# d8ahazard/AudioLab

Measured on AMD Instinct MI355X. Metric: stems*realtime-factor (44.1kHz stereo), higher is better.
Workload: dtype bf16; 1 GPU; MDX-Net UVR 4-stem (4x TFC-TDF U-Net L=11 g=48 dim_f=3072 dim_t=256 n_fft=6144), 300 s 44.1 kHz stereo in total, margin chunker, windows/launch=52; stems=4

## Files before the change

### audiolab_amd/csrc/tdfnet.hip

```cpp
#include "mma.h"
#include <alsep_gfx950_asm.h>

#include <map>

namespace {

constexpr int kThreads = 256;

template <typename T> struct Vec16;
template <> struct Vec16<float> { static constexpr int N = 4; };
template <> struct Vec16<bf16_t> { static constexpr int N = 8; };
__device__ __forceinline__ void store_vec(float* p, const float* y) { *reinterpret_cast<float4*>(p) = make_float4(y[0], y[1], y[2], y[3]); }
__device__ __forceinline__ void store_vec(bf16_t* p, const float* y) {
    bf16x8 q;
#pragma unroll
    for (int e = 0; e < 8; ++e) q[e] = (bf16_t)y[e];
    *reinterpret_cast<bf16x8*>(p) = q;
}
__device__ __forceinline__ void load_vec(const float* p, float* x) {
    const float4 q = *reinterpret_cast<const float4*>(p);
    x[0] = q.x; x[1] = q.y; x[2] = q.z; x[3] = q.w;
}
__device__ __forceinline__ void load_vec(const bf16_t* p, float* x) {
    const bf16x8 q = *reinterpret_cast<const bf16x8*>(p);
#pragma unroll
    for (int e = 0; e < 8; ++e) x[e] = (float)q[e];
}

constexpr int kFirstThreads = 192;
template <typename T>
__global__ void __launch_bounds__(kFirstThreads)
first_conv_kernel(const T* __restrict__ X, T* __restrict__ Y, const float* __restrict__ W,
                  const float* __restrict__ scale, const float* __restrict__ shift, int64_t npix, int g,
                  float in_scale) {
    constexpr int VN = Vec16<T>::N;
    const int q = g / VN;
    const int ppb = kFirstThreads / q;
    const int tg = threadIdx.x % q, tp = threadIdx.x / q;
    if (tp >= ppb) return;
    const int co = tg * VN;
    float4 w[VN];
    float sc[VN], sh[VN];
#pragma unroll
    for (int r = 0; r < VN; ++r) {
        w[r] = *reinterpret_cast<const float4*>(W + (co + r) * 4);
        sc[r] = scale[co + r] * in_scale;
        sh[r] = shift[co + r];
    }
    for (int64_t p = (int64_t)blockIdx.x * ppb + tp; p < npix; p += (int64_t)gridDim.x * ppb) {
        float x[4];
        load4(X + p * 4, x);
        float y[VN];
#pragma unroll
        for (int r = 0; r < VN; ++r) {
            float a = w[r].x * x[0];
            a = fmaf(w[r].y, x[1], a);
            a = fmaf(w[r].z, x[2], a);
            a = fmaf(w[r].w, x[3], a);
            y[r] = fmaxf(fmaf(a, sc[r], sh[r]), 0.f);
        }
        store_vec(Y + p * g + co, y);
    }
}

template <typename T>
__global__ void __launch_bounds__(kThreads)
final_conv_kernel(const T* __restrict__ X, T* __restrict__ Y, const float* __restrict__ W,
                  const float* __restrict__ bias, int64_t npix, int c, float alpha, float beta) {
    constexpr int VN = Vec16<T>::N;
    const int lane = threadIdx.x & 63, wave = threadIdx.x >> 6;
    const int gpp = c / VN;
    T* stg = reinterpret_cast<T*>(alsep_smem) + (size_t)wave * 64 * c;
    const int64_t p0 = ((int64_t)blockIdx.x * 4 + wave) * 64;
    for (int i = lane; i < 64 * gpp; i += 64) {
        const int64_t pix = p0 + i / gpp;
        vec16 v = zero16();
        if (pix < npix) v = *reinterpret_cast<const vec16*>(X + p0 * c + (int64_t)i * VN);
        *reinterpret_cast<vec16*>(stg + (size_t)i * VN) = v;
    }
    __builtin_amdgcn_wave_barrier();
    const int64_t p = p0 + lane;
    float y[4] = {bias[0], bias[1], bias[2], bias[3]};
    for (int ci = 0; ci < c; ci += VN) {
        float x[VN];
        load_vec(stg + (size_t)lane * c + ci, x);
#pragma unroll
// ... 1423 lines not shown
            wait_vmcnt<GLDS_PER_TILE>();                     \
        } else {                                                                                  \
            wait_vmcnt<0>();                                                                      \
        }                                                                                         \
        barrier_nodrain();                                        \
        compute(S_);                                                                              \
        barrier_nodrain();                                   \
    } while (0)
    issue(0, 0);
    for (int it = 0; it < ntile; it += 2) {
        ALSEP_TDF_STEP(it, 0);
        if (it + 1 < ntile) ALSEP_TDF_STEP(it + 1, 1);
    }
#undef ALSEP_TDF_STEP
    float* stg = reinterpret_cast<float*>(alsep_smem) + (size_t)wave * (64 * Tc::SS);
    float bvv[8];
#pragma unroll
    for (int mi = 0; mi < 8; ++mi) {
        const int fo = row0 + mi * 16 + l15;
        bvv[mi] = (bias && fo < M) ? bias[fo] : 0.f;
    }
    float sc[3][4], sh[3][4];
#pragma unroll
    for (int ni = 0; ni < 3; ++ni)
#pragma unroll
        for (int r = 0; r < 4; ++r) {
            sc[ni][r] = uvalid ? scale[cb + ni * 16 + 4 * lq + r] : 0.f;
            sh[ni][r] = uvalid ? shift[cb + ni * 16 + 4 * lq + r] : 0.f;
        }
#pragma unroll
    for (int half = 0; half < 2; ++half) {
#pragma unroll
        for (int ni = 0; ni < 3; ++ni)
#pragma unroll
            for (int m4 = 0; m4 < 4; ++m4) {
                const int mi = half * 4 + m4;
                float4 v;
                v.x = fmaxf(fmaf(acc[ni][mi][0] + bvv[mi], sc[ni][0], sh[ni][0]), 0.f);
                v.y = fmaxf(fmaf(acc[ni][mi][1] + bvv[mi], sc[ni][1], sh[ni][1]), 0.f);
                v.z = fmaxf(fmaf(acc[ni][mi][2] + bvv[mi], sc[ni][2], sh[ni][2]), 0.f);
                v.w = fmaxf(fmaf(acc[ni][mi][3] + bvv[mi], sc[ni][3], sh[ni][3]), 0.f);
                *reinterpret_cast<float4*>(stg + (m4 * 16 + l15) * Tc::SS + ni * 16 + 4 * lq) = v;
            }
        __builtin_amdgcn_wave_barrier();
#pragma unroll
        for (int it = 0; it < 6; ++it) {
            const int gidx = it * 64 + lane;
            const int fr = gidx / 6, cg = gidx % 6;
            const int fo = row0 + half * 64 + fr;
            const float4 lo = *reinterpret_cast<const float4*>(stg + fr * Tc::SS + cg * 8);
            const float4 hi = *reinterpret_cast<const float4*>(stg + fr * Tc::SS + cg * 8 + 4);
            if (uvalid && fo < M) {
                const int64_t o = (bt * M + fo) * (int64_t)C + cb + cg * 8;
                float y[8] = {lo.x, lo.y, lo.z, lo.w, hi.x, hi.y, hi.z, hi.w};
                if (RESIDUAL) {
                    const bf16x8 xr = *reinterpret_cast<const bf16x8*>(R + o);
#pragma unroll
                    for (int e = 0; e < 8; ++e) y[e] += (float)xr[e];
                }
                bf16x8 q;
#pragma unroll
                for (int e = 0; e < 8; ++e) q[e] = (bf16_t)y[e];
                stream_store(reinterpret_cast<bf16x8*>(Y + o), q);
            }
        }
        __builtin_amdgcn_wave_barrier();
    }
}

template <int WM>
struct TdfWide {
    static constexpr int TR = 48, BM = TR * WM, UN = 4, UC = 48, BK = 64, NST = 3;
    static constexpr int THREADS = 64 * WM;
    static constexpr int UNIT_ELEMS = BK * UC;
    static constexpr int STAGE_ELEMS = UN * UNIT_ELEMS;
    static constexpr int PIECES = STAGE_ELEMS / 8 / 64;
    static constexpr int GLDS = PIECES / WM;
    static constexpr int WLOADS = 6;
    static constexpr size_t ring_bytes = (size_t)NST * STAGE_ELEMS * sizeof(bf16_t);
    static constexpr int SS = 52;
    static constexpr size_t stage_bytes = (size_t)WM * TR * SS * sizeof(float);
    static constexpr size_t lds_bytes = ring_bytes > stage_bytes ? ring_bytes : stage_bytes;
    static_assert(PIECES % WM == 0 && 6 % GLDS == 0, "a wave's LDS-DMA pieces stay inside one unit");
};

template <int OFF>
__device__ __forceinline__ bf16x8 tdfw_read_frag(const bf16_t* base) {
    const bf16x4 lo = lds_read_tr16_b64_off<OFF>(base);
    const bf16x4 hi = lds_read_tr16_b64_off<OFF + 16 * 48 * 2>(base);
    return __builtin_shufflevector(lo, hi, 0, 1, 2, 3, 4, 5, 6, 7);
}
template <int KS, int U>
__device__ __forceinline__ void tdfw_read_x(bf16x8 (&xf)[3], const bf16_t* base) {
    constexpr int OFF = (U * 64 * 48 + KS * 32 * 48) * 2;
    xf[0] = tdfw_read_frag<OFF>(base);
    xf[1] = tdfw_read_frag<OFF + 32>(base);
    xf[2] = tdfw_read_frag<OFF + 64>(base);
}

#ifndef ALSEP_TDF_ABL
#define ALSEP_TDF_ABL 0
#endif
template <int WM, bool RESIDUAL, int RPF = 2>
__global__ void __launch_bounds__(64 * WM, 2)
tdf_bf16_wide_kernel(const bf16_t* __restrict__ X, bf16_t* __restrict__ Y, const bf16_t* __restrict__ Wf,
                     const float* __restrict__ bias, const float* __restrict__ scale, const float* __restrict__ shift,
                     const bf16_t* __restrict__ R, int M, int K, int64_t nunits, int C, int nyb) {
    typedef TdfWide<WM> Tc;
    bf16_t* ring = reinterpret_cast<bf16_t*>(alsep_smem);
    const int tid = threadIdx.x, lane = tid & 63;
    const int wave = __builtin_amdgcn_readfirstlane(tid >> 6);
    const int l15 = lane & 15, lq = lane >> 4;
    int bx = blockIdx.x, by = blockIdx.y;
    if (nyb > 0) {
        const int i = (int)blockIdx.x >> 3;
        by = i % nyb;
        bx = (i / nyb) * 8 + ((int)blockIdx.x & 7);
    }
    const int rowblk = by * WM + wave;
    const int upc = C / Tc::UC;
    const int64_t u0 = (int64_t)bx * Tc::UN;
    const int ntile = K / Tc::BK;
    if (ntile <= 0) return;

    const int du = (wave * Tc::GLDS) / 6, dp0 = (wave * Tc::GLDS) % 6;
    const int64_t dU = u0 + du;
    const char* xu = reinterpret_cast<const char*>(X + ((dU / upc) * K) * (int64_t)C + (int)(dU % upc) * Tc::UC) +
                     (size_t)(dp0 / 3) * 32 * C * sizeof(bf16_t);
    unsigned xoff[3];
#pragma unroll
    for (int j = 0; j < 3; ++j) {
        const int within = j * 64 + lane;
        xoff[j] = (unsigned)(((within / 6) * C + (within % 6) * 8) * (int)sizeof(bf16_t));
    }
    auto issue_x = [&](int it, int stage) {
        bf16_t* dst = ring + (size_t)stage * Tc::STAGE_ELEMS + (size_t)du * Tc::UNIT_ELEMS + (size_t)dp0 * 64 * 8;
        const char* xk = opaque_uniform_ptr(xu + (size_t)it * (Tc::BK * sizeof(bf16_t)) * C);
#pragma unroll
        for (int j = 0; j < Tc::GLDS; ++j)
            glds16(xk + (size_t)(j / 3) * 32 * C * sizeof(bf16_t) + xoff[j % 3], dst + (size_t)j * 64 * 8);
    };
    const char* wrow = reinterpret_cast<const char*>(Wf) + (size_t)rowblk * ntile * (Tc::WLOADS * 1024);
    const unsigned woff = (unsigned)lane * 16u;
    bf16x8 wf[2][2][3];
    auto issue_w = [&](int it, int par) {
        const char* wp = opaque_uniform_ptr(wrow + (size_t)it * (Tc::WLOADS * 1024));
        const char* wq = wp + 4096;
        global_load_async_bf16x8<0>(wf[par][0][0], wp, woff);
        global_load_async_bf16x8<1024>(wf[par][0][1], wp, woff);
        global_load_async_bf16x8<2048>(wf[par][0][2], wp, woff);
        global_load_async_bf16x8<3072>(wf[par][1][0], wp, woff);
        global_load_async_bf16x8<0>(wf[par][1][1], wq, woff);
        global_load_async_bf16x8<1024>(wf[par][1][2], wq, woff);
    };

    f32x4 acc[Tc::UN][3][3];
#pragma unroll
    for (int u = 0; u < Tc::UN; ++u)
#pragma unroll
        for (int ni = 0; ni < 3; ++ni)
#pragma unroll
            for (int mi = 0; mi < 3; ++mi) acc[u][ni][mi] = f32x4{0.f, 0.f, 0.f, 0.f};

    const int trow = l15 >> 2, tcol = (l15 & 3) * 4;
    const bf16_t* xlane = ring + (4 * lq + trow) * Tc::UC + tcol;
    auto mma_unit = [&](int u, const bf16x8 (&xf)[3], int par, int ks) {
#pragma unroll
        for (int ni = 0; ni < 3; ++ni)
#pragma unroll
            for (int mi = 0; mi < 3; ++mi) mma_step(acc[u][ni][mi], xf[ni], wf[(ALSEP_TDF_ABL & 1) ? 0 : par][ks][mi]);
    };
#define ALSEP_TDFW_STEP(it_, S_, P_)                                                              \
    do {                                                                                          \
        wait_vmcnt<Tc::GLDS>();                 \
        if ((it_) + 1 >= ntile) wait_vmcnt<0>();          \
        barrier_nodrain();                  \
        if ((it_) + 1 < ntile && !(ALSEP_TDF_ABL & 1)) issue_w((it_) + 1, 1 - (P_));              \
        if ((it_) + 2 < ntile && !(ALSEP_TDF_ABL & 4)) issue_x((it_) + 2, ((S_) + 2) % 3);        \
        const bf16_t* xs_ = xlane + (size_t)(S_) * Tc::STAGE_ELEMS;                               \
        bf16x8 xa[3], xb[3];                                                                      \
        tdfw_read_x<0, 0>(xa, xs_);                                                               \
        tdfw_read_x<0, 1>(xb, xs_);                                                               \
        lds_read_tr16_wait_n<6>();  mma_unit(0, xa, P_, 0);                                       \
        tdfw_read_x<0, 2>(xa, xs_);                                                               \
        lds_read_tr16_wait_n<6>();  mma_unit(1, xb, P_, 0);                                       \
        tdfw_read_x<0, 3>(xb, xs_);                                                               \
        lds_read_tr16_wait_n<6>();  mma_unit(2, xa, P_, 0);                                       \
        tdfw_read_x<1, 0>(xa, xs_);                                                               \
        lds_read_tr16_wait_n<6>();  mma_unit(3, xb, P_, 0);                                       \
        tdfw_read_x<1, 1>(xb, xs_);                                                               \
        lds_read_tr16_wait_n<6>();  mma_unit(0, xa, P_, 1);                                       \
        tdfw_read_x<1, 2>(xa, xs_);                                                               \
        lds_read_tr16_wait_n<6>();  mma_unit(1, xb, P_, 1);                                       \
        tdfw_read_x<1, 3>(xb, xs_);                                                               \
        lds_read_tr16_wait_n<6>();  mma_unit(2, xa, P_, 1);                                       \
        lds_read_tr16_wait_n<0>();  mma_unit(3, xb, P_, 1);                                       \
    } while (0)
    issue_x(0, 0);
    issue_w(0, 0);
    if (1 < ntile) issue_x(1, 1);
    for (int it = 0; it < ntile; it += 6) {
        ALSEP_TDFW_STEP(it, 0, 0);
        if (it + 1 < ntile) ALSEP_TDFW_STEP(it + 1, 1, 1);
        if (it + 2 < ntile) ALSEP_TDFW_STEP(it + 2, 2, 0);
        if (it + 3 < ntile) ALSEP_TDFW_STEP(it + 3, 0, 1);
        if (it + 4 < ntile) ALSEP_TDFW_STEP(it + 4, 1, 0);
        if (it + 5 < ntile) ALSEP_TDFW_STEP(it + 5, 2, 1);
    }
#undef ALSEP_TDFW_STEP
    wait_vmcnt<0>();
#pragma unroll
    for (int i = 0; i < 12; ++i) keep_vgprs_live(wf[i / 6][(i / 3) % 2][i % 3]);
    barrier_nodrain();

    float* stg = reinterpret_cast<float*>(alsep_smem) + (size_t)wave * (Tc::TR * Tc::SS);
    float bvv[3];
#pragma unroll
    for (int mi = 0; mi < 3; ++mi) bvv[mi] = bias ? bias[rowblk * Tc::TR + mi * 16 + l15] : 0.f;
    auto unit_base = [&](int u) {
        const int64_t U = u0 + u;
        return ((U / upc) * M + rowblk * Tc::TR) * (int64_t)C + (int)(U % upc) * Tc::UC;
    };
    unsigned loff[5];
#pragma unroll
    for (int it = 0; it < 5; ++it) {
        const int gidx = it * 64 + lane;
        loff[it] = (unsigned)(((gidx / 6) * C + (gidx % 6) * 8) * (int)sizeof(bf16_t));
    }
    constexpr int PF = RESIDUAL ? RPF : 0;
    bf16x8 rr[Tc::UN][5];
    auto load_res = [&](int u) {
        const ALSEP_GLOBAL char* rb = opaque_uniform_gptr(reinterpret_cast<const char*>(R + unit_base(u)));
#pragma unroll
        for (int it = 0; it < 5; ++it)
            if (it * 64 + lane < Tc::TR * 6) rr[u][it] = *reinterpret_cast<const ALSEP_GLOBAL bf16x8*>(rb + loff[it]);
    };
    if (RESIDUAL && !(ALSEP_TDF_ABL & 2)) {
#pragma unroll
        for (int u = 0; u < PF && u < Tc::UN; ++u) load_res(u);
    }
#pragma unroll
    for (int u = 0; u < Tc::UN; ++u) {
        const int cb = (int)((u0 + u) % upc) * Tc::UC;
        if (RESIDUAL && u + PF < Tc::UN && !(ALSEP_TDF_ABL & 2)) load_res(u + PF);
        ALSEP_GLOBAL char* yb = const_cast<ALSEP_GLOBAL char*>(opaque_uniform_gptr(reinterpret_cast<const char*>(Y + unit_base(u))));
#pragma unroll
        for (int ni = 0; ni < 3; ++ni) {
            const f32x4 sc = *reinterpret_cast<const f32x4*>(scale + cb + ni * 16 + 4 * lq);
            const f32x4 sh = *reinterpret_cast<const f32x4*>(shift + cb + ni * 16 + 4 * lq);
#pragma unroll
            for (int mi = 0; mi < 3; ++mi) {
                f32x4 v;
#pragma unroll
                for (int r = 0; r < 4; ++r) v[r] = fmaxf(fmaf(acc[u][ni][mi][r] + bvv[mi], sc[r], sh[r]), 0.f);
                *reinterpret_cast<f32x4*>(stg + (mi * 16 + l15) * Tc::SS + ni * 16 + 4 * lq) = v;
            }
        }
        __builtin_amdgcn_wave_barrier();
#pragma unroll
        for (int it = 0; it < 5; ++it) {
            const int gidx = it * 64 + lane;
            const int fr = gidx / 6, cg = gidx % 6;
            if (gidx < Tc::TR * 6) {
                const f32x4 lo = *reinterpret_cast<const f32x4*>(stg + fr * Tc::SS + cg * 8);
                const f32x4 hi = *reinterpret_cast<const f32x4*>(stg + fr * Tc::SS + cg * 8 + 4);
                float y[8] = {lo[0], lo[1], lo[2], lo[3], hi[0], hi[1], hi[2], hi[3]};
                if (RESIDUAL) {
#pragma unroll
                    for (int e = 0; e < 8; ++e) y[e] += (float)rr[u][it][e];
                }
                bf16x8 q;
#pragma unroll
                for (int e = 0; e < 8; ++e) q[e] = (bf16_t)y[e];
                stream_store(reinterpret_cast<ALSEP_GLOBAL bf16x8*>(yb + loff[it]), q);
            }
        }
        __builtin_amdgcn_wave_barrier();
    }
}

struct Ds48 { static constexpr int C = 48, M = 96, MS = M + 4, K = 192, MT = 6, KS = 6; };
__device__ __forceinline__ vec16 lds_read16_align8(const bf16_t* p) {
    struct alignas(8) half16 { uint32_t w[2]; };
    const half16 a = *reinterpret_cast<const half16*>(p), b = *reinterpret_cast<const half16*>(p + 4);
    vec16 v;
    v.w[0] = a.w[0]; v.w[1] = a.w[1]; v.w[2] = b.w[0]; v.w[3] = b.w[1];
    return v;
}

__global__ void __launch_bounds__(kThreads, 1)
ds48_stream_kernel(const bf16_t* __restrict__ X, bf16_t* __restrict__ Y, const bf16_t* __restrict__ Wf,
                   const float* __restrict__ scale, const float* __restrict__ shift, int64_t npix, int Tp, int Fp) {
    typedef Ds48 D;
    const int tid = threadIdx.x, lane = tid & 63, wave = tid >> 6;
    const int l15 = lane & 15, lq = lane >> 4;
    bf16_t* stg = reinterpret_cast<bf16_t*>(alsep_smem) + (size_t)wave * 64 * D::MS;
    bf16x8 wf[D::MT][D::KS];
#pragma unroll
    for (int mt = 0; mt < D::MT; ++mt)
#pragma unroll
        for (int ks = 0; ks < D::KS; ++ks)
            wf[mt][ks] = *reinterpret_cast<const bf16x8*>(Wf + ((size_t)(mt * D::KS + ks) * 64 + lane) * 8);
    float sc[D::MT][4], sh[D::MT][4];
#pragma unroll
    for (int mt = 0; mt < D::MT; ++mt)
#pragma unroll
        for (int r = 0; r < 4; ++r) { sc[mt][r] = scale[mt * 16 + 4 * lq + r]; sh[mt][r] = shift[mt * 16 + 4 * lq + r]; }
    const int64_t ntile = npix / 64;
    for (int64_t tile = (int64_t)blockIdx.x * 4 + wave; tile < ntile; tile += (int64_t)gridDim.x * 4) {
        const int64_t p0 = tile * 64;
        const int64_t fp0 = p0 % Fp, tp = (p0 / Fp) % Tp, bb = p0 / ((int64_t)Fp * Tp);
        const bf16_t* xrow = X + ((bb * 2 * Tp + 2 * tp) * (2 * (int64_t)Fp) + 2 * fp0) * D::C;
        f32x4 acc[D::MT][4];
#pragma unroll
        for (int mt = 0; mt < D::MT; ++mt)
#pragma unroll
            for (int ni = 0; ni < 4; ++ni) acc[mt][ni] = f32x4{0.f, 0.f, 0.f, 0.f};
#pragma unroll
        for (int ks = 0; ks < D::KS; ++ks) {
            const int k = ks * 32 + lq * 8;
            const int dy = k / (2 * D::C), rem = k % (2 * D::C);
            bf16x8 xf[4];
#pragma unroll
            for (int ni = 0; ni < 4; ++ni)
                xf[ni] = *reinterpret_cast<const bf16x8*>(xrow + (int64_t)dy * (2 * (int64_t)Fp * D::C) + (int64_t)(ni * 16 + l15) * (2 * D::C) + rem);
#pragma unroll
            for (int mt = 0; mt < D::MT; ++mt)
#pragma unroll
                for (int ni = 0; ni < 4; ++ni) mma_step(acc[mt][ni], wf[mt][ks], xf[ni]);
        }
#pragma unroll
        for (int mt = 0; mt < D::MT; ++mt)
#pragma unroll
            for (int ni = 0; ni < 4; ++ni) {
                float y[4];
#pragma unroll
                for (int r = 0; r < 4; ++r) y[r] = fmaxf(fmaf(acc[mt][ni][r], sc[mt][r], sh[mt][r]), 0.f);
                store4(stg + (ni * 16 + l15) * D::MS + mt * 16 + 4 * lq, y);
            }
        __builtin_amdgcn_wave_barrier();
        bf16_t* yrow = Y + p0 * D::M;
#pragma unroll
        for (int it = 0; it < 64 * D::M / 8 / 64; ++it) {
            const int gidx = it * 64 + lane;
            *reinterpret_cast<vec16*>(yrow + (size_t)gidx * 8) = lds_read16_align8(stg + (gidx / (D::M / 8)) * D::MS + (gidx % (D::M / 8)) * 8);
        }
        __builtin_amdgcn_wave_barrier();
    }
}

template <int C_> struct DsSplitCfg {
    static constexpr int C = C_, M = C_ + 48, MS = M + 4, K = 4 * C_, MT = M / 16, KS = K / 32, MTW = (MT + 3) / 4;
    static_assert(M % 16 == 0 && K % 32 == 0, "ds stream geometry");
};
template <int C_, int OCC>
__global__ void __launch_bounds__(kThreads, OCC)
ds_split_stream_kernel(const bf16_t* __restrict__ X, bf16_t* __restrict__ Y, const bf16_t* __restrict__ Wf,
                       const float* __restrict__ scale, const float* __restrict__ shift, int64_t npix, int Tp, int Fp) {
    typedef DsSplitCfg<C_> D;
    const int tid = threadIdx.x, lane = tid & 63, wave = tid >> 6;
// ... 1082 lines not shown
        note_launch(ctx, "us_stream_kernel<" #CIN_ "," #C2_ ">");                                                          \
    }
        if (L.K == 96) ALSEP_US(96, 48, 4, 1, 512)
        else if (L.K == 144) ALSEP_US(144, 96, 2, 2, 512)
        else ALSEP_US(192, 144, 2, 1, 256)
#undef ALSEP_US
    }
    note_launch(ctx, mode == PIX_DS ? "ds_stream_kernel" : "us_stream_kernel");
    ALSEP_LAUNCH_CHECK(ctx, "pix stream kernel");
    return ALSEP_OK;
}
int run_pix_stream(alsep_ctx* ctx, int, const GemmLayer&, const float*, float*, const float*, int64_t, int, int) {
    return alsep_fail(ctx, ALSEP_ERR_STATE, "streaming ds/us path is bf16 only");
}

#ifndef ALSEP_F16_TU
template <int MODE>
int run_pix_split(alsep_ctx* ctx, const GemmLayer& L, const float* X, float* Y, const float* skip, int64_t ncols, int Tp, int Fp, int C, int C2) {
    typedef GemmSCfg Gc;
    const int64_t gx = ceil_div64(ncols, Gc::BC);
    if (gx > 0x7fffffff) return alsep_fail(ctx, ALSEP_ERR_ARG, "pix_gemm: too many column tiles");
    ALSEP_HIP(ctx, hipFuncSetAttribute((const void*)pix_gemm_f32s_kernel<MODE>, hipFuncAttributeMaxDynamicSharedMemorySize, (int)Gc::lds_bytes));
    ProfScope prof(ctx, ALSEP_PROF_PIX);
    const int nrb = L.Mp / Gc::BR;
    const int fast = (nrb > 1 && gx % 8 == 0 && gx * nrb <= 0x7fffffff) ? nrb : 0;
    hipLaunchKernelGGL((pix_gemm_f32s_kernel<MODE>), fast ? dim3((unsigned)(gx * nrb)) : dim3((unsigned)gx, nrb), dim3(kThreads), Gc::lds_bytes,
                       ctx->stream, X, Y, (const hs_t*)L.w.p, (const float*)L.scale.p, (const float*)L.shift.p, skip, L.M, L.Mp, L.K, L.Kp, ncols,
                       Tp, Fp, C, C2, L.range_flag, fast);
    ALSEP_LAUNCH_CHECK(ctx, "pix_gemm_f32s_kernel");
    return ALSEP_OK;
}
template <int MODE>
int run_pix_split(alsep_ctx* ctx, const GemmLayer&, const bf16_t*, bf16_t*, const bf16_t*, int64_t, int, int, int, int) {
    return alsep_fail(ctx, ALSEP_ERR_STATE, "split contraction is a float32 mode");
}
int run_tdf_split(alsep_ctx* ctx, const GemmLayer& L, const float* X, float* Y, const float* R, int64_t BT, int C) {
    typedef GemmSCfg Gc;
    const int64_t nunits = BT * (C / 16);
    const int64_t gx = ceil_div64(nunits, 8);
    if (gx > 0x7fffffff) return alsep_fail(ctx, ALSEP_ERR_ARG, "tdf_gemm: too many column tiles");
    const float* bias = L.has_bias ? (const float*)L.bias.p : nullptr;
    ProfScope prof(ctx, ALSEP_PROF_TDF);
    const int nrb = L.Mp / Gc::BR;
    const int fast = (nrb > 1 && gx % 8 == 0 && gx * nrb <= 0x7fffffff) ? nrb : 0;
    const dim3 grid = fast ? dim3((unsigned)(gx * nrb)) : dim3((unsigned)gx, nrb);
    if (R) {
        ALSEP_HIP(ctx, hipFuncSetAttribute((const void*)tdf_gemm_f32s_kernel<true>, hipFuncAttributeMaxDynamicSharedMemorySize, (int)Gc::lds_bytes));
        hipLaunchKernelGGL((tdf_gemm_f32s_kernel<true>), grid, dim3(kThreads), Gc::lds_bytes, ctx->stream, X, Y, (const hs_t*)L.w.p, bias,
                           (const float*)L.scale.p, (const float*)L.shift.p, R, L.M, L.Mp, L.K, L.Kp, nunits, C, L.range_flag, fast);
    } else {
        ALSEP_HIP(ctx, hipFuncSetAttribute((const void*)tdf_gemm_f32s_kernel<false>, hipFuncAttributeMaxDynamicSharedMemorySize, (int)Gc::lds_bytes));
        hipLaunchKernelGGL((tdf_gemm_f32s_kernel<false>), grid, dim3(kThreads), Gc::lds_bytes, ctx->stream, X, Y, (const hs_t*)L.w.p, bias,
                           (const float*)L.scale.p, (const float*)L.shift.p, R, L.M, L.Mp, L.K, L.Kp, nunits, C, L.range_flag, fast);
    }
    ALSEP_LAUNCH_CHECK(ctx, "tdf_gemm_f32s_kernel");
    return ALSEP_OK;
}
int run_tdf_split(alsep_ctx* ctx, const GemmLayer&, const bf16_t*, bf16_t*, const bf16_t*, int64_t, int) {
    return alsep_fail(ctx, ALSEP_ERR_STATE, "split contraction is a float32 mode");
}
#endif

template <typename T, int MODE>
int run_pix(alsep_ctx* ctx, const GemmLayer& L, const T* X, T* Y, const T* skip, int64_t ncols, int Tp, int Fp, int C, int C2) {
    typedef GemmCfg<T> Gc;
#ifndef ALSEP_F16_TU
    if (L.split) return run_pix_split<MODE>(ctx, L, X, Y, skip, ncols, Tp, Fp, C, C2);
#endif
    if (L.wfrag.p && pix_stream_enabled() && Fp % 64 == 0) return run_pix_stream(ctx, MODE, L, X, Y, skip, ncols, Tp, Fp);
    const int64_t gx = ceil_div64(ncols, Gc::BC);
    if (gx > 0x7fffffff) return alsep_fail(ctx, ALSEP_ERR_ARG, "pix_gemm: too many column tiles");
    ProfScope prof(ctx, ALSEP_PROF_PIX);
    hipLaunchKernelGGL((pix_gemm_kernel<T, MODE>), dim3((unsigned)gx, L.Mp / Gc::BR), dim3(kThreads), Gc::lds_bytes,
                       ctx->stream, X, Y, (const T*)L.w.p, (const float*)L.scale.p, (const float*)L.shift.p, skip,
                       L.M, L.K, L.Kp, ncols, Tp, Fp, C, C2);
    ALSEP_LAUNCH_CHECK(ctx, "pix_gemm_kernel");
    return ALSEP_OK;
}

int tdf_wide_mode() {
    static const int v = [] { const char* e = getenv("ALSEP_TDF_WIDE"); return e ? atoi(e) : 1; }();
    return v;
}
template <int WM>
int launch_tdf_wide(alsep_ctx* ctx, const GemmLayer& L, const bf16_t* X, bf16_t* Y, const bf16_t* R, int64_t nunits, int C) {
    typedef TdfWide<WM> Tc;
    const int64_t gx = ceil_div64(nunits, Tc::UN);
    if (gx > 0x7fffffff) return alsep_fail(ctx, ALSEP_ERR_ARG, "tdf: too many column tiles");
    const float* bias = L.has_bias ? (const float*)L.bias.p : nullptr;
    static const int yfast = [] { const char* e = getenv("ALSEP_TDF_YFAST"); return e ? atoi(e) : 1; }();
    const int nrb = L.M / Tc::BM;
    const int nyb = (yfast && nrb > 1 && gx % 8 == 0 && gx * nrb <= 0x7fffffff) ? nrb : 0;
    const dim3 grid = nyb ? dim3((unsigned)(gx * nrb)) : dim3((unsigned)gx, nrb);
    ProfScope prof(ctx, ALSEP_PROF_TDF);
    static const int rpf = [] { const char* e = getenv("ALSEP_TDF_RPF"); return e ? atoi(e) : 2; }();
    if (R && rpf == 0) {
        ALSEP_HIP(ctx, hipFuncSetAttribute((const void*)tdf_bf16_wide_kernel<WM, true, 0>,
                                           hipFuncAttributeMaxDynamicSharedMemorySize, (int)Tc::lds_bytes));
        hipLaunchKernelGGL((tdf_bf16_wide_kernel<WM, true, 0>), grid, dim3(Tc::THREADS), Tc::lds_bytes, ctx->stream, X, Y,
                           (const bf16_t*)L.wwide.p, bias, (const float*)L.scale.p, (const float*)L.shift.p, R, L.M, L.K,
                           nunits, C, nyb);
    } else if (R) {
        ALSEP_HIP(ctx, hipFuncSetAttribute((const void*)tdf_bf16_wide_kernel<WM, true>,
                                           hipFuncAttributeMaxDynamicSharedMemorySize, (int)Tc::lds_bytes));
        hipLaunchKernelGGL((tdf_bf16_wide_kernel<WM, true>), grid, dim3(Tc::THREADS), Tc::lds_bytes, ctx->stream, X, Y,
                           (const bf16_t*)L.wwide.p, bias, (const float*)L.scale.p, (const float*)L.shift.p, R, L.M, L.K,
                           nunits, C, nyb);
    } else {
        ALSEP_HIP(ctx, hipFuncSetAttribute((const void*)tdf_bf16_wide_kernel<WM, false>,
                                           hipFuncAttributeMaxDynamicSharedMemorySize, (int)Tc::lds_bytes));
        hipLaunchKernelGGL((tdf_bf16_wide_kernel<WM, false>), grid, dim3(Tc::THREADS), Tc::lds_bytes, ctx->stream, X, Y,
                           (const bf16_t*)L.wwide.p, bias, (const float*)L.scale.p, (const float*)L.shift.p, R, L.M, L.K,
                           nunits, C, nyb);
    }
    note_launch(ctx, R ? "tdf_bf16_wide_kernel<res>" : "tdf_bf16_wide_kernel<nores>");
    ALSEP_LAUNCH_CHECK(ctx, "tdf_bf16_wide_kernel");
    return ALSEP_OK;
}

int run_tdf_dma(alsep_ctx* ctx, const GemmLayer& L, const bf16_t* X, bf16_t* Y, const bf16_t* R, const bf16_t* zp,
                int64_t BT, int C) {
    typedef TdfB16 Tc;
    const int64_t nunits = BT * (C / Tc::UC);
    if (L.wwide.p && tdf_wide_mode() && L.K % 64 == 0 && nunits % 4 == 0) {
        const int mode = tdf_wide_mode();
        const bool can8 = L.M % 384 == 0;
        const bool use8 = mode == 8 ? can8 : (mode == 4 ? false : (can8 && L.M == 384 && !R));
        return use8 ? launch_tdf_wide<8>(ctx, L, X, Y, R, nunits, C) : launch_tdf_wide<4>(ctx, L, X, Y, R, nunits, C);
    }
    const int64_t gx = ceil_div64(nunits, Tc::UN);
    if (gx > 0x7fffffff) return alsep_fail(ctx, ALSEP_ERR_ARG, "tdf: too many column tiles");
    const float* bias = L.has_bias ? (const float*)L.bias.p : nullptr;
    ProfScope prof(ctx, ALSEP_PROF_TDF);
    const dim3 grid((unsigned)gx, L.Mp / Tc::BM);
    if (R)
        hipLaunchKernelGGL((tdf_bf16_kernel<true>), grid, dim3(kThreads), Tc::lds_bytes, ctx->stream, X, Y, (const bf16_t*)L.w.p,
                           bias, (const float*)L.scale.p, (const float*)L.shift.p, R, zp, L.M, L.K, L.Kp, nunits, C);
    else
        hipLaunchKernelGGL((tdf_bf16_kernel<false>), grid, dim3(kThreads), Tc::lds_bytes, ctx->stream, X, Y, (const bf16_t*)L.w.p,
                           bias, (const float*)L.scale.p, (const float*)L.shift.p, R, zp, L.M, L.K, L.Kp, nunits, C);
    ALSEP_LAUNCH_CHECK(ctx, "tdf_bf16_kernel");
    return ALSEP_OK;
}
int run_tdf_dma(alsep_ctx* ctx, const GemmLayer&, const float*, float*, const float*, const float*, int64_t, int) {
    return alsep_fail(ctx, ALSEP_ERR_STATE, "LDS-DMA TDF path is bf16 only");
}

template <typename T>
int run_tdf(alsep_ctx* ctx, const GemmLayer& L, const T* X, T* Y, const T* R, int64_t BT, int C, const void* zero_page) {
    typedef GemmCfg<T> Gc;
#ifndef ALSEP_F16_TU
    if (L.split) return run_tdf_split(ctx, L, X, Y, R, BT, C);
#endif
    if (L.dma_path) return run_tdf_dma(ctx, L, X, Y, R, (const T*)zero_page, BT, C);
    const int64_t nunits = BT * (C / 16);
    const int64_t gx = ceil_div64(nunits, 8);
    if (gx > 0x7fffffff) return alsep_fail(ctx, ALSEP_ERR_ARG, "tdf_gemm: too many column tiles");
    const float* bias = L.has_bias ? (const float*)L.bias.p : nullptr;
    ProfScope prof(ctx, ALSEP_PROF_TDF);
    if (R)
        hipLaunchKernelGGL((tdf_gemm_kernel<T, true>), dim3((unsigned)gx, L.Mp / Gc::BR), dim3(kThreads), Gc::lds_bytes,
                           ctx->stream, X, Y, (const T*)L.w.p, bias, (const float*)L.scale.p, (const float*)L.shift.p, R,
                           L.M, L.K, L.Kp, nunits, C);
    else
        hipLaunchKernelGGL((tdf_gemm_kernel<T, false>), dim3((unsigned)gx, L.Mp / Gc::BR), dim3(kThreads), Gc::lds_bytes,
                           ctx->stream, X, Y, (const T*)L.w.p, bias, (const float*)L.scale.p, (const float*)L.shift.p, R,
                           L.M, L.K, L.Kp, nunits, C);
    ALSEP_LAUNCH_CHECK(ctx, "tdf_gemm_kernel");
    return ALSEP_OK;
}

template <typename T>
int run_block(alsep_ctx* ctx, const alsep_net* net, const Block& blk, const T* cur, T* a, T* b, T* h, T* dest,
              int64_t B, int Th, int Fw, int c) {
    const T* src = cur;
    T* pp[2] = {a, b};
    int rc;
    const int l = (int)blk.tfc.size();
    for (int j = 0; j < l; ++j) {
        T* dst = pp[j & 1];
        if ((rc = run_conv<T>(ctx, blk.tfc[j], src, dst, B, Th, Fw, net->zero_page.p))) return rc;
        src = dst;
    }
    if (blk.tdf.size() == 2) {
        if ((rc = run_tdf<T>(ctx, blk.tdf[0], src, h, (const T*)nullptr, B * Th, c, net->zero_page.p))) return rc;
        return run_tdf<T>(ctx, blk.tdf[1], h, dest, src, B * Th, c, net->zero_page.p);
    }
    return run_tdf<T>(ctx, blk.tdf[0], src, dest, src, B * Th, c, net->zero_page.p);
}

size_t align256(size_t v) { return (v + 255) & ~(size_t)255; }

struct WsLayout {
    size_t p0, p1, p2, h, total;
    std::vector<size_t> skip;
};

WsLayout ws_layout(const alsep_net* net, int64_t B) {
    const alsep_net_config& cfg = net->cfg;
    const size_t es = cfg.dtype == ALSEP_F32 ? 4 : 2;
    WsLayout w;
    const size_t s0 = align256((size_t)B * cfg.dim_t * cfg.dim_f * cfg.g * es);
    size_t off = 0;
    w.p0 = off; off += s0;
    w.p1 = off; off += s0;
    w.p2 = off; off += s0;
    w.h = off;  off += align256(cfg.bn > 0 ? s0 / cfg.bn : 16);
    int c = cfg.g;
    size_t t = cfg.dim_t, f = cfg.dim_f;
    for (int i = 0; i < net->n; ++i) {
        w.skip.push_back(off);
        off += align256((size_t)B * t * f * c * es);
        c += cfg.g; t /= 2; f /= 2;
    }
    w.total = off;
    return w;
}

struct PcmFront {
    const alsep_plan* plan;
    const float* pcm;
    int64_t ch_stride, chunk_stride;
    int zero_low;
};

template <typename T>
int forward_impl(alsep_ctx* ctx, const alsep_net* net, const T* in, T* out, int64_t B, char* ws, float in_scale,
                 float out_alpha, float out_beta, const PcmFront* front = nullptr) {
    const alsep_net_config& cfg = net->cfg;
    const WsLayout L = ws_layout(net, B);
    T* P[3] = {(T*)(ws + L.p0), (T*)(ws + L.p1), (T*)(ws + L.p2)};
    T* H = (T*)(ws + L.h);
    int Th = cfg.dim_t, Fw = cfg.dim_f, c = cfg.g;
    const int64_t npix0 = B * Th * Fw;
    int rc;
    if (front) {
        if ((rc = ALSEP_TU_NAME(alsep_stft_first_conv)(ctx, front->plan, front->pcm, front->ch_stride, front->chunk_stride, B, P[0],
                                                       (const float*)net->first_w.p, (const float*)net->first_scale.p,
                                                       (const float*)net->first_shift.p, cfg.g, in_scale, front->zero_low)))
            return rc;
    } else {
        ProfScope prof(ctx, ALSEP_PROF_POINTWISE);
        const int ppb = kFirstThreads / (cfg.g / Vec16<T>::N);
        const int64_t nblk = std::min<int64_t>(ceil_div64(npix0, ppb), 256 * 16);
        hipLaunchKernelGGL((first_conv_kernel<T>), dim3((unsigned)nblk), dim3(kFirstThreads), 0,
                           ctx->stream, in, P[0], (const float*)net->first_w.p, (const float*)net->first_scale.p,
                           (const float*)net->first_shift.p, npix0, cfg.g, in_scale);
        ALSEP_LAUNCH_CHECK(ctx, "first_conv_kernel");
    }
    int ic = 0;
    for (int i = 0; i < net->n; ++i) {
        T* skip = (T*)(ws + L.skip[i]);
        if ((rc = run_block<T>(ctx, net, net->enc[i], P[ic], P[(ic + 1) % 3], P[(ic + 2) % 3], H, skip, B, Th, Fw, c))) return rc;
        const int Tp = Th / 2, Fp = Fw / 2;
        if ((rc = run_pix<T, PIX_DS>(ctx, net->ds[i], skip, P[ic], (const T*)nullptr, B * Tp * Fp, Tp, Fp, c, c + cfg.g))) return rc;
        Th = Tp; Fw = Fp; c += cfg.g;
    }
    {
        T* dest = P[(ic + 1) % 3];
        if ((rc = run_block<T>(ctx, net, net->bott, P[ic], P[(ic + 2) % 3], P[ic], H, dest, B, Th, Fw, c))) return rc;
        ic = (ic + 1) % 3;
    }
    for (int i = 0; i < net->n; ++i) {
        const T* skip = (const T*)(ws + L.skip[net->n - 1 - i]);
        const int c2 = c - cfg.g;
        T* up = P[(ic + 1) % 3];
        if ((rc = run_pix<T, PIX_US>(ctx, net->us[i], P[ic], up, skip, B * Th * Fw, Th, Fw, c, c2))) return rc;
        Th *= 2; Fw *= 2; c = c2;
        T* dest = P[ic];
        if ((rc = run_block<T>(ctx, net, net->dec[i], up, P[(ic + 2) % 3], up, H, dest, B, Th, Fw, c))) return rc;
    }
    ProfScope prof(ctx, ALSEP_PROF_POINTWISE);
    hipLaunchKernelGGL((final_conv_kernel<T>), dim3((unsigned)ceil_div64(npix0, kThreads)), dim3(kThreads),
                       (size_t)kThreads * cfg.g * sizeof(T), ctx->stream,
                       (const T*)P[ic], out, (const float*)net->final_w.p, (const float*)net->final_b.p, npix0, cfg.g, out_alpha, out_beta);
    ALSEP_LAUNCH_CHECK(ctx, "final_conv_kernel");
    return ALSEP_OK;
}

}

extern "C" int alsep_net_create_f16tu(alsep_ctx*, const alsep_net_config*, const alsep_tensor*, int64_t, alsep_net**);
extern "C" int alsep_net_destroy_f16tu(alsep_net*);
extern "C" int64_t alsep_net_workspace_bytes_f16tu(const alsep_net*, int64_t);
extern "C" int alsep_net_forward_f16tu(alsep_ctx*, const alsep_net*, const void*, void*, int64_t, void*, int64_t, float, float, float);

extern "C" int ALSEP_TU_NAME(alsep_net_create)(alsep_ctx* ctx, const alsep_net_config* cfg, const alsep_tensor* tensors,
                                int64_t n_tensors, alsep_net** out) {
    ALSEP_ENTER(ctx);
#ifndef ALSEP_F16_TU
    if (ctx && cfg && cfg->dtype == ALSEP_F16) return alsep_net_create_f16tu(ctx, cfg, tensors, n_tensors, out);
#endif
    if (!ctx || !cfg || !tensors || !out) return alsep_fail(ctx, ALSEP_ERR_ARG, "alsep_net_create: null argument");
    const int n = cfg->num_blocks / 2;
    if (cfg->num_blocks < 1 || cfg->l < 1 || cfg->g < 16 || cfg->g % 16 != 0 || cfg->bn < 0 ||
        (cfg->dtype != ALSEP_F32 && cfg->dtype != ALSEP_HALF_DTYPE))
        return alsep_fail(ctx, ALSEP_ERR_ARG, "alsep_net_create: unsupported config (g must be a multiple of 16)");
    if ((cfg->flags & ~ALSEP_NET_SPLIT_F16) != 0 || ((cfg->flags & ALSEP_NET_SPLIT_F16) && cfg->dtype != ALSEP_F32))
        return alsep_fail(ctx, ALSEP_ERR_ARG, "alsep_net_create: unknown flags, or ALSEP_NET_SPLIT_F16 on a network that is not float32");
    if (cfg->dim_f % (1 << n) != 0 || cfg->dim_t % (1 << n) != 0 ||
        (cfg->bn > 0 && (cfg->dim_f >> n) % cfg->bn != 0))
        return alsep_fail(ctx, ALSEP_ERR_ARG, "alsep_net_create: dim_f/dim_t not divisible by 2^%d (and bn)", n);
    TensorMap tm;
    for (int64_t i = 0; i < n_tensors; ++i) {
        if (!tensors[i].name || !tensors[i].data || tensors[i].numel < 0)
            return alsep_fail(ctx, ALSEP_ERR_ARG, "alsep_net_create: bad tensor entry %lld", (long long)i);
        std::vector<float> h((size_t)tensors[i].numel);
        if (tensors[i].numel)
            ALSEP_HIP(ctx, hipMemcpy(h.data(), tensors[i].data, sizeof(float) * h.size(), hipMemcpyDeviceToHost));
        tm[tensors[i].name] = std::move(h);
    }
    alsep_net* net = new alsep_net();
    net->ctx = ctx;
    net->cfg = *cfg;
    net->n = n;
    net->split = cfg->dtype == ALSEP_F32 && (cfg->flags & ALSEP_NET_SPLIT_F16) != 0;
    const int rc = cfg->dtype == ALSEP_F32 ? build_net<float>(net, tm) : build_net<bf16_t>(net, tm);
    if (rc) {
        const std::string keep = ctx->err;
        ALSEP_TU_NAME(alsep_net_destroy)(net);
        ctx->err = keep;
        return rc;
    }
    *out = net;
    return ALSEP_OK;
}

extern "C" int ALSEP_TU_NAME(alsep_net_destroy)(alsep_net* net) {
    if (!net) return ALSEP_OK;
#ifndef ALSEP_F16_TU
    if (net->cfg.dtype == ALSEP_F16) return alsep_net_destroy_f16tu(net);
#endif
    for (auto& b : net->owned)
        if (b.p) (void)hipFree(b.p);
    delete net;
    return ALSEP_OK;
}

extern "C" int64_t ALSEP_TU_NAME(alsep_net_workspace_bytes)(const alsep_net* net, int64_t B) {
    if (!net || B <= 0) return 0;
#ifndef ALSEP_F16_TU
    if (net->cfg.dtype == ALSEP_F16) return alsep_net_workspace_bytes_f16tu(net, B);
#endif
    return (int64_t)ws_layout(net, B).total;
}

extern "C" int ALSEP_TU_NAME(alsep_net_forward)(alsep_ctx* ctx, const alsep_net* net, const void* spec_in, void* spec_out,
                                 int64_t B, void* workspace, int64_t workspace_bytes, float in_scale,
                                 float out_alpha, float out_beta) {
    ALSEP_ENTER(ctx);
#ifndef ALSEP_F16_TU
    if (net && net->cfg.dtype == ALSEP_F16)
        return alsep_net_forward_f16tu(ctx, net, spec_in, spec_out, B, workspace, workspace_bytes, in_scale, out_alpha, out_beta);
#endif
// ... 50 lines not shown
```

Measured before the change: 5809 stems*x_realtime.

## Fold final 1x1 output conv into last decoder TDF residual GEMM epilogue

Adds a FINAL variant of the wide TDF kernel that, for the last decoder block, keeps the bf16 residual-added rows in LDS instead of writing them to global memory. It then computes the 4-channel final pointwise conv per row, using weights staged in LDS, and writes the scaled output directly. This is meant to remove the full-resolution activation write plus the separate final_conv_kernel launch and its reread. In exchange the epilogue does extra per-lane FMA work, leaves the Y buffer unwritten, and only applies when C equals 48, WM is 4 and out_beta is zero.

```diff
diff --git a/audiolab_amd/csrc/tdfnet.hip b/audiolab_amd/csrc/tdfnet.hip
--- a/audiolab_amd/csrc/tdfnet.hip
+++ b/audiolab_amd/csrc/tdfnet.hip
@@ -2,6 +2,7 @@
 #include <alsep_gfx950_asm.h>
 
 #include <map>
+#include <type_traits>
 
 namespace {
 
@@ -1591,6 +1592,9 @@
     static constexpr size_t stage_bytes = (size_t)WM * TR * SS * sizeof(float);
     static constexpr size_t lds_bytes = ring_bytes > stage_bytes ? ring_bytes : stage_bytes;
     static_assert(PIECES % WM == 0 && 6 % GLDS == 0, "a wave's LDS-DMA pieces stay inside one unit");
+    static constexpr int FS = 56;
+    static constexpr size_t final_bytes = (size_t)WM * TR * FS * sizeof(bf16_t);
+    static constexpr int FWN = 192;
 };
 
 template <int OFF>
@@ -1610,12 +1614,15 @@
 #ifndef ALSEP_TDF_ABL
 #define ALSEP_TDF_ABL 0
 #endif
-template <int WM, bool RESIDUAL, int RPF = 2>
+template <int WM, bool RESIDUAL, int RPF = 2, bool FINAL = false>
 __global__ void __launch_bounds__(64 * WM, 2)
 tdf_bf16_wide_kernel(const bf16_t* __restrict__ X, bf16_t* __restrict__ Y, const bf16_t* __restrict__ Wf,
                      const float* __restrict__ bias, const float* __restrict__ scale, const float* __restrict__ shift,
-                     const bf16_t* __restrict__ R, int M, int K, int64_t nunits, int C, int nyb) {
+                     const bf16_t* __restrict__ R, int M, int K, int64_t nunits, int C, int nyb,
+                     const float* __restrict__ FW, const float* __restrict__ FB, bf16_t* __restrict__ FOUT, float falpha) {
     typedef TdfWide<WM> Tc;
+    static_assert(!FINAL || (RESIDUAL && Tc::stage_bytes + Tc::final_bytes + WM * Tc::FWN * sizeof(float) <= Tc::lds_bytes),
+                  "FINAL: rounded rows and the final weights behind the staging rows");
     bf16_t* ring = reinterpret_cast<bf16_t*>(alsep_smem);
     const int tid = threadIdx.x, lane = tid & 63;
     const int wave = __builtin_amdgcn_readfirstlane(tid >> 6);
@@ -1723,6 +1730,15 @@
     barrier_nodrain();
 
     float* stg = reinterpret_cast<float*>(alsep_smem) + (size_t)wave * (Tc::TR * Tc::SS);
+    bf16_t* frow = reinterpret_cast<bf16_t*>(alsep_smem + Tc::stage_bytes) + (size_t)wave * (Tc::TR * Tc::FS);
+    float* fwl = reinterpret_cast<float*>(alsep_smem + Tc::stage_bytes + Tc::final_bytes) + wave * Tc::FWN;
+    float fw[3], fbs[4];
+    if (FINAL) {
+#pragma unroll
+        for (int j = 0; j < 3; ++j) fw[j] = FW[j * 64 + lane];
+#pragma unroll
+        for (int r = 0; r < 4; ++r) fbs[r] = FB[r];
+    }
     float bvv[3];
 #pragma unroll
     for (int mi = 0; mi < 3; ++mi) bvv[mi] = bias ? bias[rowblk * Tc::TR + mi * 16 + l15] : 0.f;
@@ -1746,7 +1762,13 @@
     };
     if (RESIDUAL && !(ALSEP_TDF_ABL & 2)) {
 #pragma unroll
-        for (int u = 0; u < PF && u < Tc::UN; ++u) load_res(u);
+        for (int u = 0; u < PF && u < Tc::UN; ++u) {
+            load_res(u);
+            if (FINAL && u == 0) {
+#pragma unroll
+                for (int j = 0; j < 3; ++j) fwl[j * 64 + lane] = fw[j];
+            }
+        }
     }
 #pragma unroll
     for (int u = 0; u < Tc::UN; ++u) {
@@ -1781,10 +1803,32 @@
                 bf16x8 q;
 #pragma unroll
                 for (int e = 0; e < 8; ++e) q[e] = (bf16_t)y[e];
-                stream_store(reinterpret_cast<ALSEP_GLOBAL bf16x8*>(yb + loff[it]), q);
+                if (FINAL) *reinterpret_cast<bf16x8*>(frow + fr * Tc::FS + cg * 8) = q;
+                else stream_store(reinterpret_cast<ALSEP_GLOBAL bf16x8*>(yb + loff[it]), q);
             }
         }
         __builtin_amdgcn_wave_barrier();
+        if (FINAL) {
+            const int frl = lane < Tc::TR ? lane : Tc::TR - 1;
+            float y[4] = {fbs[0], fbs[1], fbs[2], fbs[3]};
+#pragma unroll 2
+            for (int ci = 0; ci < Tc::UC; ci += 8) {
+                const bf16x8 xv = *reinterpret_cast<const bf16x8*>(frow + frl * Tc::FS + ci);
+#pragma unroll
+                for (int r = 0; r < 4; ++r) {
+                    const f32x4 w0 = *reinterpret_cast<const f32x4*>(fwl + r * Tc::UC + ci);
+                    const f32x4 w1 = *reinterpret_cast<const f32x4*>(fwl + r * Tc::UC + ci + 4);
+#pragma unroll
+                    for (int e = 0; e < 4; ++e) y[r] = fmaf(w0[e], (float)xv[e], y[r]);
+#pragma unroll
+                    for (int e = 0; e < 4; ++e) y[r] = fmaf(w1[e], (float)xv[4 + e], y[r]);
+                }
+            }
+#pragma unroll
+            for (int r = 0; r < 4; ++r) y[r] *= falpha;
+            if (lane < Tc::TR) store4(FOUT + (((u0 + u) * M + rowblk * Tc::TR + lane) << 2), y);
+            __builtin_amdgcn_wave_barrier();
+        }
     }
 }
 
@@ -3033,8 +3077,20 @@
     static const int v = [] { const char* e = getenv("ALSEP_TDF_WIDE"); return e ? atoi(e) : 1; }();
     return v;
 }
+struct FinalFold {
+    const float* w;
+    const float* b;
+    void* out;
+    float alpha;
+    bool done;
+};
+int tdf_final_mode() {
+    static const int v = [] { const char* e = getenv("ALSEP_TDF_FINAL"); return e ? atoi(e) : 1; }();
+    return v;
+}
 template <int WM>
-int launch_tdf_wide(alsep_ctx* ctx, const GemmLayer& L, const bf16_t* X, bf16_t* Y, const bf16_t* R, int64_t nunits, int C) {
+int launch_tdf_wide(alsep_ctx* ctx, const GemmLayer& L, const bf16_t* X, bf16_t* Y, const bf16_t* R, int64_t nunits, int C,
+                    FinalFold* fin) {
     typedef TdfWide<WM> Tc;
     const int64_t gx = ceil_div64(nunits, Tc::UN);
     if (gx > 0x7fffffff) return alsep_fail(ctx, ALSEP_ERR_ARG, "tdf: too many column tiles");
@@ -3045,24 +3101,32 @@
     const dim3 grid = nyb ? dim3((unsigned)(gx * nrb)) : dim3((unsigned)gx, nrb);
     ProfScope prof(ctx, ALSEP_PROF_TDF);
     static const int rpf = [] { const char* e = getenv("ALSEP_TDF_RPF"); return e ? atoi(e) : 2; }();
-    if (R && rpf == 0) {
+    if (WM == 4 && R && rpf != 0 && fin && C == Tc::UC && tdf_final_mode()) {
+        ALSEP_HIP(ctx, hipFuncSetAttribute((const void*)tdf_bf16_wide_kernel<4, true, 2, true>,
+                                           hipFuncAttributeMaxDynamicSharedMemorySize, (int)TdfWide<4>::lds_bytes));
+        hipLaunchKernelGGL((tdf_bf16_wide_kernel<4, true, 2, true>), grid, dim3(TdfWide<4>::THREADS), TdfWide<4>::lds_bytes,
+                           ctx->stream, X, Y, (const bf16_t*)L.wwide.p, bias, (const float*)L.scale.p, (const float*)L.shift.p, R,
+                           L.M, L.K, nunits, C, nyb, fin->w, fin->b, (bf16_t*)fin->out, fin->alpha);
+        fin->done = true;
+        note_launch(ctx, "tdf_bf16_wide_kernel<res,final>");
+    } else if (R && rpf == 0) {
         ALSEP_HIP(ctx, hipFuncSetAttribute((const void*)tdf_bf16_wide_kernel<WM, true, 0>,
                                            hipFuncAttributeMaxDynamicSharedMemorySize, (int)Tc::lds_bytes));
         hipLaunchKernelGGL((tdf_bf16_wide_kernel<WM, true, 0>), grid, dim3(Tc::THREADS), Tc::lds_bytes, ctx->stream, X, Y,
                            (const bf16_t*)L.wwide.p, bias, (const float*)L.scale.p, (const float*)L.shift.p, R, L.M, L.K,
-                           nunits, C, nyb);
+                           nunits, C, nyb, (const float*)nullptr, (const float*)nullptr, (bf16_t*)nullptr, 0.f);
     } else if (R) {
         ALSEP_HIP(ctx, hipFuncSetAttribute((const void*)tdf_bf16_wide_kernel<WM, true>,
                                            hipFuncAttributeMaxDynamicSharedMemorySize, (int)Tc::lds_bytes));
         hipLaunchKernelGGL((tdf_bf16_wide_kernel<WM, true>), grid, dim3(Tc::THREADS), Tc::lds_bytes, ctx->stream, X, Y,
                            (const bf16_t*)L.wwide.p, bias, (const float*)L.scale.p, (const float*)L.shift.p, R, L.M, L.K,
-                           nunits, C, nyb);
+                           nunits, C, nyb, (const float*)nullptr, (const float*)nullptr, (bf16_t*)nullptr, 0.f);
     } else {
         ALSEP_HIP(ctx, hipFuncSetAttribute((const void*)tdf_bf16_wide_kernel<WM, false>,
                                            hipFuncAttributeMaxDynamicSharedMemorySize, (int)Tc::lds_bytes));
         hipLaunchKernelGGL((tdf_bf16_wide_kernel<WM, false>), grid, dim3(Tc::THREADS), Tc::lds_bytes, ctx->stream, X, Y,
                            (const bf16_t*)L.wwide.p, bias, (const float*)L.scale.p, (const float*)L.shift.p, R, L.M, L.K,
-                           nunits, C, nyb);
+                           nunits, C, nyb, (const float*)nullptr, (const float*)nullptr, (bf16_t*)nullptr, 0.f);
     }
     note_launch(ctx, R ? "tdf_bf16_wide_kernel<res>" : "tdf_bf16_wide_kernel<nores>");
     ALSEP_LAUNCH_CHECK(ctx, "tdf_bf16_wide_kernel");
@@ -3070,14 +3134,14 @@
 }
 
 int run_tdf_dma(alsep_ctx* ctx, const GemmLayer& L, const bf16_t* X, bf16_t* Y, const bf16_t* R, const bf16_t* zp,
-                int64_t BT, int C) {
+                int64_t BT, int C, FinalFold* fin) {
     typedef TdfB16 Tc;
     const int64_t nunits = BT * (C / Tc::UC);
     if (L.wwide.p && tdf_wide_mode() && L.K % 64 == 0 && nunits % 4 == 0) {
         const int mode = tdf_wide_mode();
         const bool can8 = L.M % 384 == 0;
         const bool use8 = mode == 8 ? can8 : (mode == 4 ? false : (can8 && L.M == 384 && !R));
-        return use8 ? launch_tdf_wide<8>(ctx, L, X, Y, R, nunits, C) : launch_tdf_wide<4>(ctx, L, X, Y, R, nunits, C);
+        return use8 ? launch_tdf_wide<8>(ctx, L, X, Y, R, nunits, C, nullptr) : launch_tdf_wide<4>(ctx, L, X, Y, R, nunits, C, fin);
     }
     const int64_t gx = ceil_div64(nunits, Tc::UN);
     if (gx > 0x7fffffff) return alsep_fail(ctx, ALSEP_ERR_ARG, "tdf: too many column tiles");
@@ -3093,17 +3157,18 @@
     ALSEP_LAUNCH_CHECK(ctx, "tdf_bf16_kernel");
     return ALSEP_OK;
 }
-int run_tdf_dma(alsep_ctx* ctx, const GemmLayer&, const float*, float*, const float*, const float*, int64_t, int) {
+int run_tdf_dma(alsep_ctx* ctx, const GemmLayer&, const float*, float*, const float*, const float*, int64_t, int, FinalFold*) {
     return alsep_fail(ctx, ALSEP_ERR_STATE, "LDS-DMA TDF path is bf16 only");
 }
 
 template <typename T>
-int run_tdf(alsep_ctx* ctx, const GemmLayer& L, const T* X, T* Y, const T* R, int64_t BT, int C, const void* zero_page) {
+int run_tdf(alsep_ctx* ctx, const GemmLayer& L, const T* X, T* Y, const T* R, int64_t BT, int C, const void* zero_page,
+            FinalFold* fin = nullptr) {
     typedef GemmCfg<T> Gc;
 #ifndef ALSEP_F16_TU
     if (L.split) return run_tdf_split(ctx, L, X, Y, R, BT, C);
 #endif
-    if (L.dma_path) return run_tdf_dma(ctx, L, X, Y, R, (const T*)zero_page, BT, C);
+    if (L.dma_path) return run_tdf_dma(ctx, L, X, Y, R, (const T*)zero_page, BT, C, fin);
     const int64_t nunits = BT * (C / 16);
     const int64_t gx = ceil_div64(nunits, 8);
     if (gx > 0x7fffffff) return alsep_fail(ctx, ALSEP_ERR_ARG, "tdf_gemm: too many column tiles");
@@ -3123,7 +3188,7 @@
 
 template <typename T>
 int run_block(alsep_ctx* ctx, const alsep_net* net, const Block& blk, const T* cur, T* a, T* b, T* h, T* dest,
-              int64_t B, int Th, int Fw, int c) {
+              int64_t B, int Th, int Fw, int c, FinalFold* fin = nullptr) {
     const T* src = cur;
     T* pp[2] = {a, b};
     int rc;
@@ -3135,9 +3200,9 @@
     }
     if (blk.tdf.size() == 2) {
         if ((rc = run_tdf<T>(ctx, blk.tdf[0], src, h, (const T*)nullptr, B * Th, c, net->zero_page.p))) return rc;
-        return run_tdf<T>(ctx, blk.tdf[1], h, dest, src, B * Th, c, net->zero_page.p);
-    }
-    return run_tdf<T>(ctx, blk.tdf[0], src, dest, src, B * Th, c, net->zero_page.p);
+        return run_tdf<T>(ctx, blk.tdf[1], h, dest, src, B * Th, c, net->zero_page.p, fin);
+    }
+    return run_tdf<T>(ctx, blk.tdf[0], src, dest, src, B * Th, c, net->zero_page.p, fin);
 }
 
 size_t align256(size_t v) { return (v + 255) & ~(size_t)255; }
@@ -3199,6 +3264,8 @@
                            (const float*)net->first_shift.p, npix0, cfg.g, in_scale);
         ALSEP_LAUNCH_CHECK(ctx, "first_conv_kernel");
     }
+    FinalFold fold = {(const float*)net->final_w.p, (const float*)net->final_b.p, out, out_alpha, false};
+    FinalFold* const fin = (!std::is_same<T, float>::value && out_beta == 0.f) ? &fold : nullptr;
     int ic = 0;
     for (int i = 0; i < net->n; ++i) {
         T* skip = (T*)(ws + L.skip[i]);
@@ -3209,7 +3276,8 @@
     }
     {
         T* dest = P[(ic + 1) % 3];
-        if ((rc = run_block<T>(ctx, net, net->bott, P[ic], P[(ic + 2) % 3], P[ic], H, dest, B, Th, Fw, c))) return rc;
+        if ((rc = run_block<T>(ctx, net, net->bott, P[ic], P[(ic + 2) % 3], P[ic], H, dest, B, Th, Fw, c, net->n == 0 ? fin : nullptr)))
+            return rc;
         ic = (ic + 1) % 3;
     }
     for (int i = 0; i < net->n; ++i) {
@@ -3219,8 +3287,10 @@
         if ((rc = run_pix<T, PIX_US>(ctx, net->us[i], P[ic], up, skip, B * Th * Fw, Th, Fw, c, c2))) return rc;
         Th *= 2; Fw *= 2; c = c2;
         T* dest = P[ic];
-        if ((rc = run_block<T>(ctx, net, net->dec[i], up, P[(ic + 2) % 3], up, H, dest, B, Th, Fw, c))) return rc;
-    }
+        if ((rc = run_block<T>(ctx, net, net->dec[i], up, P[(ic + 2) % 3], up, H, dest, B, Th, Fw, c, i == net->n - 1 ? fin : nullptr)))
+            return rc;
+    }
+    if (fold.done) return ALSEP_OK;
     ProfScope prof(ctx, ALSEP_PROF_POINTWISE);
     hipLaunchKernelGGL((final_conv_kernel<T>), dim3((unsigned)ceil_div64(npix0, kThreads)), dim3(kThreads),
                        (size_t)kThreads * cfg.g * sizeof(T), ctx->stream,
```

Result: faster. 5878 stems*x_realtime (median of 6 runs) (+1.2%).
